# burakcuhadar/Photometric-Bundle-Adjustment

Hardware: AMD Instinct MI355X
Metric: photometric residual+jacobian blocks/sec (higher is better)
Workload: dtype f32; 1 GPU; C4: one synthetic problem of 1000 host keyframes x 100000 points x 8-px patch x 4 targets = 400000 residual blocks, 752x480 u8 images, pinhole; one step = full r + tangent-J evaluation (Ceres-mode records) at a new HBM-resident state; keyframes=1000, points=100000, patch=8, targets_per_point=4, blocks_total=400000, blocks_rank0=400000, parallelism=host-keyframe shards x1 (evaluation: no data-path collective; GN: one GPU)

## Files before the change

photometric-bundle-adjustment_amd/csrc/pba_engine.hip:

```cpp
#include <hip/hip_runtime.h>

#include <algorithm>
#include <chrono>
#include <cmath>
#include <cstdio>
#include <cstring>
#include <string>
#include <vector>

#include "pba_internal.h"
#include "pba_record.h"

using namespace pba;
using namespace pba::detail;

namespace pba {
namespace detail {
thread_local std::string g_last_error;
}
}

namespace {

__device__ __forceinline__ void make_pair(const double* __restrict__ poses, const int* __restrict__ pair_host,
// ... 530 lines not shown
  PBA_HIP(hipMemcpyAsync(e->block_point.p, block_point, n_blocks * sizeof(int), hipMemcpyHostToDevice, e->stream));
  PBA_HIP(hipMemcpyAsync(e->block_pair.p, pair_of.data(), n_blocks * sizeof(int), hipMemcpyHostToDevice, e->stream));
  std::vector<int2> pp(n_blocks);
  for (int b = 0; b < n_blocks; ++b) pp[b] = make_int2(block_point[b], pair_of[b]);
  PBA_HIP(e->block_pp.upload(pp, e->stream));
  PBA_HIP(hipMemcpyAsync(e->pair_host.p, ph.data(), np * sizeof(int), hipMemcpyHostToDevice, e->stream));
  PBA_HIP(hipMemcpyAsync(e->pair_target.p, pt.data(), np * sizeof(int), hipMemcpyHostToDevice, e->stream));
  if (geometric) {
    PBA_HIP(e->u_obs.resize(n_blocks));
    PBA_HIP(hipMemcpyAsync(e->u_obs.p, u_obs, n_blocks * sizeof(double2), hipMemcpyHostToDevice, e->stream));
  }
  PBA_HIP(e->out.resize((size_t)n_blocks * rec));
  PBA_HIP(e->cost.resize(n_blocks));
  PBA_HIP(e->valid.resize(n_blocks));
  PBA_HIP(hipStreamSynchronize(e->stream));
  e->n_blocks = n_blocks;
  e->n_pairs = np;
  e->evaluated = false;
  e->res_fresh = false;
  e->chunk_blocks = 0;
  e->n_chunks_async = 0;
  e->chunks_arrived.store(0);
  e->pairs_fresh = false;
  e->block_point_h.assign(block_point, block_point + n_blocks);
  e->block_target_h.assign(block_target, block_target + n_blocks);
  e->pair_of_h = std::move(pair_of);
  e->pair_host_h = std::move(ph);
  e->pair_target_h = std::move(pt);
  e->gn.prepared = false;
  e->aff.planned = false;
  e->aff.linearized = e->aff.have_step = false;
  e->joint.planned = e->joint.linearized = false;
  return upload_block_records(e);
}

int pba_set_state(pba_engine* e, const double* poses, const double* inv_dist) {
  if (!e || !poses || !inv_dist) return fail(PBA_ERR_INVALID_ARGUMENT, "null state");
  if (e->n_points <= 0 || e->n_frames <= 0) return fail(PBA_ERR_NOT_READY, "problem not set");
  if (int rc = check_device(e)) return rc;
  PBA_HIP(e->poses.resize(7 * (size_t)e->n_frames));
  PBA_HIP(hipMemcpyAsync(e->poses.p, poses, 7 * (size_t)e->n_frames * sizeof(double), hipMemcpyHostToDevice, e->stream));
  PBA_HIP(hipMemcpyAsync(e->rho.p, inv_dist, (size_t)e->n_points * sizeof(double), hipMemcpyHostToDevice, e->stream));
  e->state_set = true;
  e->pairs_fresh = false;
  e->joint.linearized = false;
  return PBA_OK;
}

int pba_set_state_device(pba_engine* e, const double* d_poses, const double* d_inv_dist) {
  if (!e || !d_poses || !d_inv_dist) return fail(PBA_ERR_INVALID_ARGUMENT, "null state");
  if (e->n_points <= 0 || e->n_frames <= 0) return fail(PBA_ERR_NOT_READY, "problem not set");
  if (int rc = check_device(e)) return rc;
  PBA_HIP(e->poses.resize(7 * (size_t)e->n_frames));
  const int n_pose_d = 7 * e->n_frames;
  const bool table = e->n_blocks > 0 && e->opt.residual_kind == PBA_RESIDUAL_GEOMETRIC;
  const int pair_wgs = table ? (e->n_pairs + 255) / 256 : 0;
  const int copy_wgs = std::min(1024, (std::max(n_pose_d, e->n_points) + 255) / 256);
  state_kernel<<<pair_wgs + copy_wgs, 256, 0, e->stream>>>(d_poses, d_inv_dist, e->poses.p, e->rho.p, n_pose_d,
                                                           e->n_points, e->pair_host.p, e->pair_target.p,
                                                           e->frame_cam.p, e->intr_d.p, e->pairs.p, e->n_pairs,
                                                           pair_wgs);
  PBA_HIP(hipGetLastError());
  e->state_set = true;
  e->pairs_fresh = table;
  e->joint.linearized = false;
  return PBA_OK;
}

namespace {

int evaluate_at(pba_engine* e, const double* poses, const double* rho, bool adopt, bool jac) {
  const bool photometric = e->opt.residual_kind == PBA_RESIDUAL_PHOTOMETRIC;
  if (photometric && (!e->have_images || e->P <= 0)) return fail(PBA_ERR_NOT_READY, "images/pattern missing");
  if (int rc = check_device(e)) return rc;
  KernelArgs ka;
  if (photometric) {
    const long long lanes = (long long)e->n_blocks * 8;
    if (adopt && lanes < std::max<long long>(7LL * e->n_frames, e->n_points)) {
      if (int rc = pba_set_state_device(e, poses, rho)) return rc;
      poses = e->poses.p;
      rho = e->rho.p;
      adopt = false;
    }
    ka = make_kernel_args(e, nullptr, rho);
    ka.poses = poses;
    if (adopt) {
      PBA_HIP(e->poses.resize(7 * (size_t)e->n_frames));
      ka.adopt_poses = e->poses.p;
      ka.adopt_rho = e->rho.p;
      e->state_set = true;
      e->pairs_fresh = false;
    }
  } else {
    if (adopt) {
      if (int rc = pba_set_state_device(e, poses, rho)) return rc;
    } else if (!e->pairs_fresh) {
      launch_pairs(e, e->poses.p, e->pairs.p);
    }
    e->pairs_fresh = true;
    ka = make_kernel_args(e, e->pairs.p, e->rho.p);
  }
  hipEvent_t ev_stop = nullptr;
  if (e->timing) {
    while (e->ev_pool.size() < e->ev_used + 2) {
      hipEvent_t ev;
      PBA_HIP(hipEventCreateWithFlags(&ev, hipEventDisableSystemFence));
      e->ev_pool.push_back(ev);
    }
    PBA_HIP(hipEventRecord(e->ev_pool[e->ev_used], e->stream));
    ev_stop = e->ev_pool[e->ev_used + 1];
    e->ev_used += 2;
  }
  if (!jac) {
    PBA_HIP(e->res.resize((size_t)e->n_blocks * e->R()));
    ka.res_out = e->res.p;
  }
  launch_mode(e, ka, jac ? 1 : 0);
  PBA_HIP(hipGetLastError());
  if (ev_stop) PBA_HIP(hipEventRecord(ev_stop, e->stream));
  e->evaluated = true;
  e->res_fresh = !jac;
  e->chunk_blocks = 0;
  e->n_chunks_async = 0;
  e->chunks_arrived.store(0);
  return PBA_OK;
}

}

int pba_evaluate(pba_engine* e, int32_t want_jacobians) {
  if (!e) return fail(PBA_ERR_INVALID_ARGUMENT, "null engine");
  if (e->n_blocks <= 0) return fail(PBA_ERR_NOT_READY, "pba_set_blocks first");
  if (!e->state_set) return fail(PBA_ERR_NOT_READY, "pba_set_state first");
  return evaluate_at(e, e->poses.p, e->rho.p, false, want_jacobians != 0);
}

int pba_evaluate_state_device(pba_engine* e, const double* d_poses, const double* d_inv_dist, int32_t want_jacobians) {
  if (!e || !d_poses || !d_inv_dist) return fail(PBA_ERR_INVALID_ARGUMENT, "null state");
  if (e->n_blocks <= 0) return fail(PBA_ERR_NOT_READY, "pba_set_blocks first");
  return evaluate_at(e, d_poses, d_inv_dist, true, want_jacobians != 0);
}

int pba_evaluate_states_device(pba_engine* e, int32_t n, const double* const* d_poses, const double* const* d_inv_dist,
                               int32_t want_jacobians) {
  if (!e || n < 0 || (n > 0 && (!d_poses || !d_inv_dist))) return fail(PBA_ERR_INVALID_ARGUMENT, "null states");
  if (e->n_blocks <= 0) return fail(PBA_ERR_NOT_READY, "pba_set_blocks first");
  for (int i = 0; i < n; ++i) {
    if (!d_poses[i] || !d_inv_dist[i]) return fail(PBA_ERR_INVALID_ARGUMENT, "null state");
    if (int rc = evaluate_at(e, d_poses[i], d_inv_dist[i], true, want_jacobians != 0)) return rc;
  }
  return PBA_OK;
}

int pba_enable_kernel_timing(pba_engine* e, int32_t enable) {
  if (!e) return fail(PBA_ERR_INVALID_ARGUMENT, "null engine");
  e->timing = enable != 0;
  return PBA_OK;
}

int pba_get_kernel_timing(pba_engine* e, double* total_ms, int32_t* launches) {
  if (!e || !total_ms) return fail(PBA_ERR_INVALID_ARGUMENT, "null argument");
  if (int rc = check_device(e)) return rc;
  PBA_HIP(hipStreamSynchronize(e->stream));
  double tot = 0;
  for (size_t i = 0; i + 1 < e->ev_used; i += 2) {
    float ms = 0;
    PBA_HIP(hipEventElapsedTime(&ms, e->ev_pool[i], e->ev_pool[i + 1]));
    tot += ms;
// ... 246 lines not shown
```

photometric-bundle-adjustment_amd/csrc/pba_evaluate.hip:

```cpp
#include <hip/hip_runtime.h>

#include <cmath>
#include <type_traits>

#include "pba_internal.h"
#include "pba_record.h"

using namespace pba;
using namespace pba::detail;

namespace {

template <int PM, int LPB, int MODE, class T>
__global__ __launch_bounds__(kBlockThreads) void photometric_block_kernel(const KernelArgs a) {
  constexpr int BPW = kBlockThreads / LPB;
  constexpr bool JAC = MODE == 1;
  using S = typename RecFormat<T>::S;
  constexpr int kCols = RecFormat<T>::kCols;
  constexpr int kStageBytes = JAC ? BPW * kCols * LPB * (int)sizeof(S) : 0;
  constexpr int kTileBytes = BPW * (int)sizeof(TileBlock);
  __shared__ __attribute__((aligned(16))) unsigned char lds[kStageBytes > kTileBytes ? kStageBytes : kTileBytes];
  TileBlock* s_tb = reinterpret_cast<TileBlock*>(lds);
  const int P = a.P;
  const int rec_f = kCols * P;
  const int blk0 = logical_tile() * BPW;
  const int lb = threadIdx.x / LPB;
  const int k = threadIdx.x % LPB;
  const int blk = blk0 + lb;
  const bool live = blk < a.n_blocks;
  const bool act = live && k < P;
  S* out = reinterpret_cast<S*>(a.out);

  const float2 off = pattern_at<LPB>(a, k);
  adopt_state(a);
  int pt;
  if (LPB == 8 && a.poses) {
    static_assert(kBlockThreads == 256, "stage_tile_wg: 4 waves, 32 blocks");
    pt = a.block_rec[live ? blk : a.n_blocks - 1].x;
    stage_tile_wg(a, s_tb, blk0);
  } else {
    pt = stage_tile<LPB>(a, s_tb, lb, k, blk, live);
  }
  const float Ih = act ? a.host_int[(long long)pt * P + k] : 0.0f;
  constexpr bool AFF = RecFormat<T>::kAffine;
  Affine af = {1.0f, 0.0f, 0.0f};
  if constexpr (AFF) af = block_affine(a, live ? blk : a.n_blocks - 1);
  __syncthreads();
  constexpr bool INTR = JAC && RecFormat<T>::kIntr;
  constexpr bool PFIN = RecFormat<T>::kIntr && AFF;
  float ji[8];
  const Row row = photometric_row<PM, JAC, TileBlock, false, INTR, AFF, PFIN>(a, s_tb[lb], off, Ih, nullptr, ji, &af);
  const int ok = group_all<LPB>(act ? row.ok : 1);
  const float s = group_sum<LPB>(act ? row.r * row.r : 0.0f);
  const float bc = ok ? huber_cost(s, a.huber) : 0.0f;
  if (live && k == 0) {
    a.valid[blk] = (uint8_t)ok;
    a.cost[blk] = bc;
  }
  if (MODE == 2) {
    if (a.wg_red) {
      const bool one = live && k == 0;
      wg_reduce2(one ? (double)bc : 0.0, one && ok ? 1.0 : 0.0, a.wg_red + 2 * logical_tile());
    }
    return;
  }
  if (!JAC) {
    if (act) {
      out[(long long)blk * rec_f + k] = rec_val<S>(ok ? row.r : 0.0f);
      if (a.res_out) a.res_out[(long long)blk * P + k] = ok ? row.r : 0.0f;
    }
    return;
  }
  __syncthreads();
  S* s_rec = reinterpret_cast<S*>(lds) + lb * rec_f;
  if constexpr (RecFormat<T>::kScaled) {
    stage_row_scaled(s_rec, lb, P, k, row, act && ok);
    if (act && !ok) {
      s_rec[k] = s_rec[col_jrho(P) + k] = s_rec[col_tail(P) + k] = (S)0.0f;
      for (int j = 0; j < 6; ++j) s_rec[col_jhost(P) + 6 * k + j] = s_rec[col_jtarget(P) + 6 * k + j] = (S)0.0f;
    }
  } else if (act) {
    if (ok) {
      stage_row_each<S>(s_rec, P, k, row);
    } else {
      S* h = s_rec + col_jhost(P) + 6 * k;
      S* t = s_rec + col_jtarget(P) + 6 * k;
      s_rec[k] = (S)0.0f;
      for (int j = 0; j < 6; ++j) h[j] = t[j] = (S)0.0f;
      s_rec[col_jrho(P) + k] = (S)0.0f;
    }
    if constexpr (INTR) {
      if (!ok) {
#pragma unroll
        for (int j = 0; j < 8; ++j) ji[j] = 0.0f;
      }
      stage_intr(s_rec, P, k, ji);
    }
    if constexpr (AFF) stage_affine<RecFormat<T>::kIntr>(s_rec, P, k, af.E * (Ih - af.bh), af.E, ok != 0);
  }
  __syncthreads();
  const int nblk = min(BPW, a.n_blocks - blk0);
  if (nblk <= 0) return;
  store_slab<S>(lds, reinterpret_cast<unsigned char*>(out + (long long)blk0 * rec_f), nblk * rec_f * (int)sizeof(S),
                a.slab_wt);
}

__host__ __device__ constexpr int multi_stage_bytes(int bpw, int P, int tsize, int cols = 14) {
  return (bpw * cols * P * tsize + 15) & ~15;
}

template <int PPL, class T>
constexpr int kMultiThreads = 32 * RecFormat<T>::kCols * 8 * PPL * (int)sizeof(typename RecFormat<T>::S) +
                                          32 * (int)sizeof(TileBlock) > 60 * 1024 ? 128 : 256;

template <int PPL, class T>
constexpr int kMultiWaves =
    RecFormat<T>::kIntr || RecFormat<T>::kAffine ? 3 : (RecFormat<T>::kScaled && PPL != 3 ? 5 : 6);
template <int PM, int PPL, class T>
constexpr int kMultiWavesPM = RecFormat<T>::kAffine && cam_of(PM) == CAM_KB4 ? 2 : kMultiWaves<PPL, T>;

template <int PM, int MODE, class T, int PPL, bool CT = false, bool C1 = false>
__global__ __launch_bounds__((kMultiThreads<PPL, T>))
__attribute__((amdgpu_waves_per_eu(CT ? (kMultiWavesPM<PM, PPL, T>) : 1, 8)))
void photometric_block_kernel_multi(const KernelArgs a) {
  constexpr int LPB = 8, NTH = kMultiThreads<PPL, T>, BPW = NTH / LPB;
  constexpr bool JAC = MODE == 1;
  static_assert(!CT || NTH == 256, "camera table: the workgroup-cooperative prologue");
  using TB = typename std::conditional<CT, TileBlockC, TileBlock>::type;
  extern __shared__ __attribute__((aligned(16))) unsigned char lds[];
  __shared__ float2 s_pat[LPB * PPL];
  __shared__ CamRec s_cam[CT ? kCamTab : 1];
  using S = typename RecFormat<T>::S;
  constexpr int kCols = RecFormat<T>::kCols;
  const int P = a.P;
  S* stage = reinterpret_cast<S*>(lds);
  TB* s_tb = reinterpret_cast<TB*>(lds + (JAC ? multi_stage_bytes(BPW, P, (int)sizeof(S), kCols) : 0));
  const int rec_f = kCols * P;
  const int blk0 = logical_tile() * BPW;
  const int lb = threadIdx.x / LPB;
  const int k = threadIdx.x % LPB;
  const int blk = blk0 + lb;
  const bool live = blk < a.n_blocks;
  S* out = reinterpret_cast<S*>(a.out);

  if ((int)threadIdx.x < LPB * PPL) s_pat[threadIdx.x] = pattern_at<LPB * PPL>(a, threadIdx.x);
  adopt_state(a);
  int pt;
  if constexpr (CT) {
    pt = a.block_rec[live ? blk : a.n_blocks - 1].x;
    stage_tile_wg_ct(a, s_tb, s_cam, a.n_cams, blk0);
  } else if (NTH == 256 && a.poses) {
    pt = a.block_rec[live ? blk : a.n_blocks - 1].x;
    stage_tile_wg(a, s_tb, blk0);
  } else {
    pt = stage_tile<LPB>(a, s_tb, lb, k, blk, live);
  }
  float Ih[PPL];
#pragma unroll
  for (int j = 0; j < PPL; ++j) {
    const int px = k + LPB * j;
    Ih[j] = live && px < P ? a.host_int[(long long)pt * P + px] : 0.0f;
  }
  constexpr bool AFF = RecFormat<T>::kAffine;
  Affine af = {1.0f, 0.0f, 0.0f};
  if constexpr (AFF) af = block_affine(a, live ? blk : a.n_blocks - 1);
  __syncthreads();
  S* s_rec = stage + lb * rec_f;
  int okl = 1;
  float s = 0.0f, rr[PPL];
  auto pixel = [&](int j, float ih) {
    const int px = k + LPB * j;
    const bool act = live && px < P;
    constexpr bool INTR = JAC && RecFormat<T>::kIntr;
    constexpr bool PFIN = RecFormat<T>::kIntr && AFF;
    float ji[8];
    const Row row =
        photometric_row<PM, JAC, TB, C1, INTR, AFF, PFIN>(a, s_tb[lb], s_pat[px < P ? px : 0], ih, s_cam, ji, &af);
    okl &= act ? row.ok : 1;
    s += act ? row.r * row.r : 0.0f;
    if constexpr (JAC && RecFormat<T>::kScaled) stage_row_scaled(s_rec, lb, P, px, row, act);
    else if constexpr (JAC) stage_row<S>(s_rec, P, px, row, act);
    if constexpr (INTR) {
      if (act) stage_intr(s_rec, P, px, ji);
    }
    if constexpr (JAC && AFF) {
      if (act) stage_affine<RecFormat<T>::kIntr>(s_rec, P, px, af.E * (ih - af.bh), af.E, true);
    }
// ... 168 lines not shown
  if ((reinterpret_cast<uintptr_t>(dst) & 15) == 0) {
    f32x4* d4 = reinterpret_cast<f32x4*>(dst);
    for (int i = threadIdx.x; i < (n_out >> 2); i += kBlockThreads)
      __builtin_nontemporal_store(f32x4{value(4 * i), value(4 * i + 1), value(4 * i + 2), value(4 * i + 3)}, d4 + i);
    for (int i = (n_out & ~3) + threadIdx.x; i < n_out; i += kBlockThreads) dst[i] = value(i);
  } else {
    for (int i = threadIdx.x; i < n_out; i += kBlockThreads) dst[i] = value(i);
  }
}

template <int MODEL>
void launch_geometric(pba_engine* e, const KernelArgs& ka, int mode) {
  const int grid = (e->n_blocks + kBlockThreads - 1) / kBlockThreads;
  e->last_grid = grid;
  if (mode == 1 && e->opt_intr) geometric_block_kernel<MODEL, true, true><<<grid, kBlockThreads, 0, e->stream>>>(ka);
  else if (mode == 1) geometric_block_kernel<MODEL, true, false><<<grid, kBlockThreads, 0, e->stream>>>(ka);
  else if (e->opt_intr) geometric_block_kernel<MODEL, false, true><<<grid, kBlockThreads, 0, e->stream>>>(ka);
  else geometric_block_kernel<MODEL, false, false><<<grid, kBlockThreads, 0, e->stream>>>(ka);
}

template <class T>
struct Tag { using type = T; };
template <int M>
using Mode = std::integral_constant<int, M>;

template <class F>
void dispatch_format(const pba_engine* e, int mode, F&& fn) {
  auto modes = [&](auto tag) {
    if (mode == 1) fn(tag, Mode<1>{});
    else if (mode == 0) fn(tag, Mode<0>{});
    else if constexpr (RecFormat<typename decltype(tag)::type>::kAffine) fn(Tag<AffineF32>{}, Mode<2>{});
    else fn(Tag<float>{}, Mode<2>{});
  };
  if (e->affine && e->opt_intr) modes(Tag<IntrAffineF32>{});
  else if (e->affine) modes(Tag<AffineF32>{});
  else if (e->opt_intr) modes(Tag<IntrF32>{});
  else if (e->record_format == PBA_RECORD_F16_SCALED) modes(Tag<ScaledF16>{});
  else if (e->record_format == PBA_RECORD_F16) modes(Tag<_Float16>{});
  else modes(Tag<float>{});
}

template <int PM, int M, class T>
void launch_block(pba_engine* e, KernelArgs ka) {
  const int grid = (int)(((long long)e->n_blocks * 8 + kBlockThreads - 1) / kBlockThreads);
  e->last_grid = grid;
  ka.slab_wt = grid <= kSlabWtGrid;
  photometric_block_kernel<PM, 8, M, T><<<grid, kBlockThreads, 0, e->stream>>>(ka);
}

template <int PM, int PPL, int M, class T>
void launch_multi(pba_engine* e, const KernelArgs& ka) {
  constexpr int nth = kMultiThreads<PPL, T>;
  const int grid = (int)(((long long)e->n_blocks * 8 + nth - 1) / nth);
  e->last_grid = grid;
  const size_t stage =
      M == 1 ? multi_stage_bytes(nth / 8, e->P, (int)sizeof(typename RecFormat<T>::S), RecFormat<T>::kCols) : 0;
  if constexpr (M == 1 && nth == 256) {
    if (ka.poses != nullptr && ka.n_cams <= kCamTab) {
      const size_t lds = stage + (size_t)(nth / 8) * sizeof(TileBlockC);
      if (ka.n_cams == 1) photometric_block_kernel_multi<PM, M, T, PPL, true, true><<<grid, nth, lds, e->stream>>>(ka);
      else photometric_block_kernel_multi<PM, M, T, PPL, true><<<grid, nth, lds, e->stream>>>(ka);
      return;
    }
  }
  photometric_block_kernel_multi<PM, M, T, PPL>
      <<<grid, nth, stage + (size_t)(nth / 8) * sizeof(TileBlock), e->stream>>>(ka);
}

template <int PM>
void launch_photometric(pba_engine* e, const KernelArgs& ka, int mode) {
  const int ppl = (e->P + 7) / 8;
  dispatch_format(e, mode, [&](auto tag, auto m) {
    using T = typename decltype(tag)::type;
    constexpr int M = decltype(m)::value;
    if (ppl <= 1) launch_block<PM, M, T>(e, ka);
    else if (ppl == 2) launch_multi<PM, 2, M, T>(e, ka);
    else if (ppl == 3) launch_multi<PM, 3, M, T>(e, ka);
    else launch_multi<PM, 4, M, T>(e, ka);
  });
}

}

namespace pba {
namespace detail {

void launch_mode(pba_engine* e, const KernelArgs& ka, int mode) {
  if (e->opt.residual_kind == PBA_RESIDUAL_GEOMETRIC) {
    switch (e->opt.camera_model) {
      case PBA_CAMERA_PINHOLE: launch_geometric<CAM_PINHOLE>(e, ka, mode); break;
      case PBA_CAMERA_DOUBLE_SPHERE: launch_geometric<CAM_DS>(e, ka, mode); break;
      case PBA_CAMERA_EUCM: launch_geometric<CAM_EUCM>(e, ka, mode); break;
      default: launch_geometric<CAM_KB4>(e, ka, mode); break;
    }
    return;
  }
  dispatch_pm(e, [&](auto pm) { launch_photometric<decltype(pm)::value>(e, ka, mode); });
}

KernelArgs make_kernel_args(pba_engine* e, const PairRec* pairs, const double* rho) {
  KernelArgs ka{};
  ka.images = e->images.p;
  ka.width = e->width;
  ka.height = e->height;
  ka.tiles_x = tiles_x_of(e->width);
  ka.frame_stride = tiled_frame_bytes(e->width, e->height);
  ka.umax = e->width + 1.0;
  ka.vmax = e->height + 1.0;
  ka.intr = e->intr.p;
  ka.intr_d = e->intr_d.p;
  ka.intr_t = e->opt_intr ? e->intr_state.p : e->intr.p;
  ka.intr_t_d = e->opt_intr ? e->intr_state_d.p : e->intr_d.p;
  ka.intr_scale = std::ldexp(1.0f, -e->level);
  ka.block_point = e->block_point.p;
  ka.block_pair = e->block_pair.p;
  ka.block_pp = e->block_pp.p;
  ka.pairs = pairs;
  ka.block_rec = e->block_rec.p;
  ka.n_pose_d = 7 * e->n_frames;
  ka.n_points = e->n_points;
  ka.u_ref = e->u_ref.p;
  ka.host_int = e->host_int.p;
  ka.rho = rho;
  ka.u_obs = e->u_obs.p;
  if (e->affine) ka.affine = e->affine_state.p;
  ka.out = e->out.p;
  ka.cost = e->cost.p;
  ka.valid = e->valid.p;
  ka.n_blocks = e->n_blocks;
  ka.n_cams = e->n_cams;
  ka.P = e->opt.residual_kind == PBA_RESIDUAL_PHOTOMETRIC ? e->P : 2;
  ka.huber = e->opt.huber_width;
  for (size_t i = 0; i < e->pattern_h.size() && i < 2 * PBA_MAX_PATTERN; ++i) ka.pattern[i] = e->pattern_h[i];
  return ka;
}

int launch_cost_only(pba_engine* e, const PairRec* pairs, const double* rho, double* wg_red, int* n_slots,
                     const double* poses, const float* intr_t, const double* intr_t_d, const double* affine) {
  KernelArgs ka = make_kernel_args(e, pairs, rho);
  ka.poses = poses;
  if (affine && e->affine) ka.affine = affine;
  if (intr_t) ka.intr_t = intr_t;
  if (intr_t_d) ka.intr_t_d = intr_t_d;
  ka.wg_red = wg_red;
  launch_mode(e, ka, 2);
  if (n_slots) *n_slots = e->last_grid;
  PBA_HIP(hipGetLastError());
  return PBA_OK;
}

int launch_decode_records(pba_engine* e, float* d_out) {
  if (e->record_format == PBA_RECORD_F32) {
    PBA_HIP(hipMemcpyAsync(d_out, e->out.p, (size_t)e->n_blocks * e->rec_floats() * sizeof(float),
                           hipMemcpyDeviceToDevice, e->stream));
    return PBA_OK;
  }
  const int grid = (e->n_blocks + kDecodeBlocks - 1) / kDecodeBlocks;
  const bool scaled = e->record_format == PBA_RECORD_F16_SCALED;
  decode_records_kernel<<<grid, kBlockThreads, 0, e->stream>>>(
      reinterpret_cast<const _Float16*>(e->out.p), d_out, e->n_blocks, e->P,
      scaled ? (int)RecFormat<ScaledF16>::kCols : (int)RecFormat<_Float16>::kCols);
  PBA_HIP(hipGetLastError());
  return PBA_OK;
}

}
// ... 2 lines not shown
```

photometric-bundle-adjustment_amd/csrc/pba_internal.h:

```cpp
#pragma once

#include <hip/hip_runtime.h>

#include <algorithm>
#include <cstdint>
#include <cstdlib>
#include <type_traits>
#include <string>
#include <vector>

#include "pba.h"
#include "pba_device.h"
#include "pba_host.h"

namespace pba {
namespace detail {

inline const char* test_hook(const char* name) {
#ifdef PBA_TEST_HOOKS
  return std::getenv(name);
#else
  (void)name;
  return nullptr;
#endif
// ... 307 lines not shown
  return ((m >> sh) & grp) == grp;
}

struct Row {
  float r = 0.0f, jr = 0.0f;
  Vec3 hv = {0, 0, 0}, hw = {0, 0, 0}, tv = {0, 0, 0}, tw = {0, 0, 0};
  int ok = 1;
};

template <int LPB>
__device__ __forceinline__ int stage_tile_pp(const KernelArgs& a, TileBlock* s_tb, int lb, int k, int2 pp);
template <int LPB>
__device__ __forceinline__ int stage_tile(const KernelArgs& a, TileBlock* s_tb, int lb, int k, int blk, bool live) {
  uint4* dst = reinterpret_cast<uint4*>(s_tb + lb);
  if (LPB >= 8 && a.poses) {
    static_assert(kCamK == 8, "fused prologue: 8 camera parts");
    const int4 br = a.block_rec[live ? blk : a.n_blocks - 1];
    const double* H = a.poses + 7 * br.y;
    const double* T = a.poses + 7 * br.z;
    double h[7], t[7];
#pragma unroll
    for (int j = 0; j < 7; ++j) {
      h[j] = H[j];
      t[j] = T[j];
    }
    const int hc = br.w >> 16, tc = br.w & 0xffff, kc = k & 7;
    const uint4 cam = reinterpret_cast<const uint4*>(kc < 4 ? a.intr_d + kCamD * hc + kCamHk : a.intr_t_d + kCamD * tc)[kc & 3];
    const uint4 ur = reinterpret_cast<const uint4*>(a.u_ref)[br.x];
    const double rho = a.rho[br.x];
    asm volatile("" ::"v"(cam.x), "v"(cam.y), "v"(cam.z), "v"(cam.w), "v"(ur.x), "v"(ur.y), "v"(ur.z), "v"(ur.w),
                 "v"(rho));
#pragma unroll
    for (int j = 0; j < 7; ++j) asm volatile("" ::"v"(h[j]), "v"(t[j]));
    PairRec& pr = s_tb[lb].pr;
    if (k < 8) dst[(int)(offsetof(PairRec, hk) / 16) + k] = cam;
    if (k >= 4 && k < 8) camera_kf_part(cam, k - 4, pr.kf);
    if (k == 0) {
      pair_rotation(h, t, pr);
    } else if (k == 1) {
      pair_translation(h, t, pr);
      pr.host_cam = hc;
      pr.target_cam = tc;
      pr.target = br.z;
      pr.host = br.y;
    } else if (k == 2) {
      dst[kPairParts] = ur;
    } else if (k == 3) {
      const long long img = (long long)br.z * a.frame_stride;
      dst[kPairParts + 1] = make_uint4(__double2loint(rho), __double2hiint(rho), (unsigned)img, (unsigned)(img >> 32));
    }
    return br.x;
  }
  return stage_tile_pp<LPB>(a, s_tb, lb, k, a.block_pp[live ? blk : a.n_blocks - 1]);
}

template <int LPB>
__device__ __forceinline__ int stage_tile_pp(const KernelArgs& a, TileBlock* s_tb, int lb, int k, int2 pp) {
  constexpr int NP = (kTileParts + LPB - 1) / LPB;
  uint4* dst = reinterpret_cast<uint4*>(s_tb + lb);
  const uint4* src = reinterpret_cast<const uint4*>(a.pairs + pp.y);
  uint4 v[NP];
#pragma unroll
  for (int i = 0; i < NP; ++i) {
    const int part = k + LPB * i;
    v[i] = part == kPairParts ? reinterpret_cast<const uint4*>(a.u_ref)[pp.x] : src[part < kPairParts ? part : 0];
  }
  const double r = a.rho[pp.x];
  const int tgt = a.pairs[pp.y].target;
  asm volatile("" ::"v"(r), "v"(tgt));
#pragma unroll
  for (int i = 0; i < NP; ++i) asm volatile("" ::"v"(v[i].x), "v"(v[i].y), "v"(v[i].z), "v"(v[i].w));
#pragma unroll
  for (int i = 0; i < NP; ++i) {
    const int part = k + LPB * i;
    if (part == kPairParts + 1) {
      const long long img = (long long)tgt * a.frame_stride;
      v[i] = make_uint4(__double2loint(r), __double2hiint(r), (unsigned)img, (unsigned)(img >> 32));
    }
    if (part < kTileParts) dst[part] = v[i];
  }
  return pp.x;
}

__device__ __forceinline__ void stage_tile_wg(const KernelArgs& a, TileBlock* s_tb, int blk0) {
  const int w = threadIdx.x >> 6, lane = threadIdx.x & 63, b = lane & 31;
  const int4 br = a.block_rec[min(blk0 + b, a.n_blocks - 1)];
  PairRec& pr = s_tb[b].pr;
  uint4* dst = reinterpret_cast<uint4*>(s_tb + b);
  if (w == 0) {
    if (lane < 32) {
      const double* H = a.poses + 7 * br.y;
      const double* T = a.poses + 7 * br.z;
      double h[4], t[4];
#pragma unroll
      for (int j = 0; j < 4; ++j) {
        h[j] = H[j];
        t[j] = T[j];
      }
      pair_rotation(h, t, pr);
    }
  } else if (w == 1) {
    if (lane < 32) {
      const double* H = a.poses + 7 * br.y;
      const double* T = a.poses + 7 * br.z;
      double h[7], t[7];
#pragma unroll
      for (int j = 0; j < 7; ++j) {
        h[j] = H[j];
        t[j] = T[j];
      }
      pair_translation(h, t, pr);
      pr.host_cam = br.w >> 16;
      pr.target_cam = br.w & 0xffff;
      pr.target = br.z;
      pr.host = br.y;
    }
  } else if (w == 2) {
    const bool tgt = lane >= 32;
    const uint4* src = reinterpret_cast<const uint4*>(tgt ? a.intr_t_d + kCamD * (br.w & 0xffff) : a.intr_d + kCamD * (br.w >> 16) + kCamHk);
    uint4 c[4];
#pragma unroll
    for (int q = 0; q < 4; ++q) c[q] = src[q];
    uint4* d = dst + (int)(offsetof(PairRec, hk) / 16) + (tgt ? 4 : 0);
#pragma unroll
    for (int q = 0; q < 4; ++q) d[q] = c[q];
    if (tgt) {
#pragma unroll
      for (int q = 0; q < 4; ++q) camera_kf_part(c[q], q, pr.kf);
    }
  } else {
    if (lane < 32) {
      dst[kPairParts] = reinterpret_cast<const uint4*>(a.u_ref)[br.x];
    } else {
      const double rho = a.rho[br.x];
      const long long img = (long long)br.z * a.frame_stride;
      dst[kPairParts + 1] = make_uint4(__double2loint(rho), __double2hiint(rho), (unsigned)img, (unsigned)(img >> 32));
    }
  }
}

__device__ __forceinline__ void stage_tile_wg_ct(const KernelArgs& a, TileBlockC* s_tb, CamRec* s_cam, int n_cams,
                                                 int blk0) {
  const int w = threadIdx.x >> 6, lane = threadIdx.x & 63, b = lane & 31;
  const int4 br = a.block_rec[min(blk0 + b, a.n_blocks - 1)];
  TileBlockC& tb = s_tb[b];
  if (w == 0) {
    if (lane < 32) {
      const double* H = a.poses + 7 * br.y;
      const double* T = a.poses + 7 * br.z;
      double h[4], t[4];
#pragma unroll
      for (int j = 0; j < 4; ++j) {
        h[j] = H[j];
        t[j] = T[j];
      }
      pair_rotation(h, t, tb);
    }
  } else if (w == 1) {
    if (lane < 32) {
      const double* H = a.poses + 7 * br.y;
      const double* T = a.poses + 7 * br.z;
      double h[7], t[7];
#pragma unroll
      for (int j = 0; j < 7; ++j) {
        h[j] = H[j];
        t[j] = T[j];
      }
      pair_translation(h, t, tb);
      tb.host_cam = br.w >> 16;
      tb.target_cam = br.w & 0xffff;
      tb.target = br.z;
      tb.host = br.y;
    }
  } else if (w == 2) {
    const int c = lane >> 3, q = lane & 7;
    if (c < n_cams) {
      const uint4 v = reinterpret_cast<const uint4*>(q < 4 ? a.intr_d + kCamD * c + kCamHk : a.intr_t_d + kCamD * c)[q & 3];
      uint4* d = reinterpret_cast<uint4*>(s_cam + c);
      d[q] = v;
      if (q >= 4) camera_kf_part(v, q - 4, s_cam[c].kf);
    }
  } else {
    if (lane < 32) {
      tb.ur = a.u_ref[br.x];
    } else {
      tb.rho = a.rho[br.x];
      tb.img = (long long)br.z * a.frame_stride;
    }
  }
}

template <int N>
__device__ __forceinline__ float2 pattern_at(const KernelArgs& a, int k) {
  float2 o = make_float2(a.pattern[0], a.pattern[1]);
#pragma unroll
  for (int j = 1; j < N; ++j)
    if (k == j) o = make_float2(a.pattern[2 * j], a.pattern[2 * j + 1]);
  return o;
}

__device__ __forceinline__ void adopt_state(const KernelArgs& a) {
  if (!a.adopt_rho) return;
  const long long g = (long long)blockIdx.x * blockDim.x + threadIdx.x;
  if (g >= a.n_points && g >= a.n_pose_d) return;
  const double r = a.rho[g < a.n_points ? g : 0], p = a.poses[g < a.n_pose_d ? g : 0];
  asm volatile("" ::"v"(r), "v"(p));
  if (g < a.n_points) a.adopt_rho[g] = r;
  if (g < a.n_pose_d) a.adopt_poses[g] = p;
}

struct Affine {
  float E, bh, bt;
};
__device__ __forceinline__ Affine block_affine(const KernelArgs& a, int blk, int pair = -1) {
  int h, t;
  if (pair < 0 && a.poses) {
    const int4 br = a.block_rec[blk];
    h = br.y;
    t = br.z;
  } else {
    const PairRec& pr = a.pairs[pair >= 0 ? pair : a.block_pp[blk].y];
    h = pr.host;
    t = pr.target;
  }
  const double2 ah = reinterpret_cast<const double2*>(a.affine)[h];
  const double2 at = reinterpret_cast<const double2*>(a.affine)[t];
  const double d = at.x - ah.x;
  const double E = isfinite(ah.x) && isfinite(at.x) ? exp(d) : __builtin_nan("");
  return {(float)E, (float)ah.y, (float)at.y};
}

template <int PM, bool JAC, class TB = TileBlock, bool C1 = false, bool INTR = false, bool AFF = false,
          bool PFIN = false>
__device__ __forceinline__ Row photometric_row(const KernelArgs& a, const TB& tb, float2 off, float Ih,
                                               const CamRec* tab = nullptr, float* ji = nullptr,
                                               const Affine* af = nullptr) {
  constexpr int MODEL = cam_of(PM);
  Row o;
  const auto& pp = pose_of(tb);
  const CamView cv = C1 ? single_camera(a) : cams_of(tb, tab);
  const double rho = tb.rho;
  const Vec3d b = unproject<MODEL>(cv.hk, tb.ur.x + (double)off.x, tb.ur.y + (double)off.y);
  const Vec3d Rb = mat_mul(pp.R, b);
  const Vec3d p = {Rb.x + rho * pp.t[0], Rb.y + rho * pp.t[1], Rb.z + rho * pp.t[2]};
  const bool dom = in_domain<MODEL>(cv.tk, p);
  float I, gx, gy;
  double u, v;
  const double iden = project<MODEL>(cv.tk, p, u, v);
  interpolate<interp_of(PM)>(a.images + tb.img, a.umax, a.vmax, a.tiles_x, u, v, I, gx, gy);
  if (AFF) o.r = (I - af->bt) - af->E * (Ih - af->bh);
  else o.r = I - Ih;
  o.ok = dom && isfinite(o.r);
  if constexpr (PFIN) o.ok = o.ok && isfinite(u) && isfinite(v);
  if (JAC) {
    const Vec3 pf = to_f(p), bf = to_f(b);
    Vec3 du, dv;
    project_jac<MODEL>(cv.kf, pf, (float)iden, du, dv);
    const Vec3 q = {gx * du.x + gy * dv.x, gx * du.y + gy * dv.y, gx * du.z + gy * dv.z};
    const Vec3 qR = row_mul(q, pp.Rf);
    const float rf = (float)rho;
    o.hv = {rf * qR.x, rf * qR.y, rf * qR.z};
    o.hw = cross(bf, qR);
    o.tv = {-rf * q.x, -rf * q.y, -rf * q.z};
    o.tw = cross(q, pf);
    if (MODEL == CAM_PINHOLE) {
      const double ex = fma(-(p.x * iden), pp.t[2], pp.t[0]), ey = fma(-(p.y * iden), pp.t[2], pp.t[1]);
      o.jr = (float)(iden * fma((double)gx * cv.tk[0], ex, (double)gy * cv.tk[1] * ey));
    } else {
      Vec3d dud, dvd;
      project_jac<MODEL>(cv.tk, p, iden, dud, dvd);
      const Vec3d td = {pp.t[0], pp.t[1], pp.t[2]};
      o.jr = (float)((double)gx * dot(dud, td) + (double)gy * dot(dvd, td));
    }
    if (INTR) {
      float ku[8], kv[8];
      if (MODEL == CAM_KB4)
        project_intr_jac_kb4(cv.kf, pf, (float)iden, (float)atan2(sqrt(p.x * p.x + p.y * p.y), p.z), ku, kv);
      else
        project_intr_jac<MODEL>(cv.kf, pf, (float)iden, ku, kv);
#pragma unroll
      for (int j = 0; j < 8; ++j) ji[j] = (gx * ku[j] + gy * kv[j]) * (j < 4 ? a.intr_scale : 1.0f);
// ... 418 lines not shown
```

photometric-bundle-adjustment_amd/csrc/pba_record.h:

```cpp
#pragma once

#include <type_traits>

#include "pba_internal.h"

namespace {

struct ScaledF16 {};
struct IntrF32 {};
struct AffineF32 {};
struct IntrAffineF32 {};
template <class Stored, int Cols, bool Scaled = false, bool Intr = false, bool Affine = false>
struct RecLayout {
  using S = Stored;
  static constexpr int kCols = Cols;
  static constexpr bool kScaled = Scaled, kIntr = Intr, kAffine = Affine;
};
template <class T>
struct RecFormat : RecLayout<T, 14> {};
template <>
struct RecFormat<ScaledF16> : RecLayout<_Float16, 15, true> {};
template <>
struct RecFormat<IntrF32> : RecLayout<float, 22, false, true> {};
template <>
struct RecFormat<AffineF32> : RecLayout<float, 18, false, false, true> {};
template <>
struct RecFormat<IntrAffineF32> : RecLayout<float, 26, false, true, true> {};

}

namespace pba {
namespace detail {

__host__ __device__ __forceinline__ constexpr int col_r(int) { return 0; }
__host__ __device__ __forceinline__ constexpr int col_jhost(int P) { return P; }
__host__ __device__ __forceinline__ constexpr int col_jtarget(int P) { return 7 * P; }
__host__ __device__ __forceinline__ constexpr int col_jrho(int P) { return 13 * P; }
__host__ __device__ __forceinline__ constexpr int col_tail(int P) { return 14 * P; }
template <bool INTR = false>
__host__ __device__ __forceinline__ constexpr int col_jab_host(int P) {
  if constexpr (INTR) return col_tail(P) + 8 * P;
  else return col_tail(P);
}
template <bool INTR = false>
__host__ __device__ __forceinline__ constexpr int col_jab_target(int P) {
  if constexpr (INTR) return col_tail(P) + 10 * P;
  else return col_tail(P) + 2 * P;
}

__host__ __device__ __forceinline__ constexpr int scale_row_of(int c, int P) {
  return c < col_jhost(P) ? -1 : c < col_jrho(P) ? ((c - col_jhost(P)) % (6 * P)) / 6 : c - col_jrho(P);
}

template <class T>
__device__ __forceinline__ T rec_val(float v) { return (T)v; }
template <>
__device__ __forceinline__ _Float16 rec_val<_Float16>(float v) {
  return (_Float16)(isnan(v) ? v : __builtin_amdgcn_fmed3f(v, -65504.0f, 65504.0f));
}

template <bool INTR = false>
__device__ __forceinline__ void stage_affine(float* s_rec, int P, int px, float g, float E, bool ok) {
  reinterpret_cast<float2*>(s_rec + col_jab_host<INTR>(P))[px] = ok ? make_float2(g, E) : make_float2(0.0f, 0.0f);
  reinterpret_cast<float2*>(s_rec + col_jab_target<INTR>(P))[px] = ok ? make_float2(-g, -1.0f) : make_float2(0.0f, 0.0f);
}

__device__ __forceinline__ void stage_intr(float* s_rec, int P, int px, const float (&ji)[8]) {
  float* d = s_rec + col_tail(P) + 8 * px;
  if ((P & 1) == 0) {
    reinterpret_cast<f32x4*>(d)[0] = f32x4{ji[0], ji[1], ji[2], ji[3]};
    reinterpret_cast<f32x4*>(d)[1] = f32x4{ji[4], ji[5], ji[6], ji[7]};
  } else {
#pragma unroll
    for (int q = 0; q < 4; ++q) reinterpret_cast<float2*>(d)[q] = make_float2(ji[2 * q], ji[2 * q + 1]);
  }
}

template <class T, int NTH = kBlockThreads>
__device__ __forceinline__ void store_slab(const unsigned char* src, unsigned char* dst, int bytes, int wt = 0) {
  constexpr int kBlockThreads = NTH;
  if ((((uintptr_t)dst | (unsigned)bytes) & 15) == 0) {
    const f32x4* s4 = reinterpret_cast<const f32x4*>(src);
    f32x4* d4 = reinterpret_cast<f32x4*>(dst);
    if (wt) {
      for (int i = threadIdx.x; i < (bytes >> 4); i += kBlockThreads)
        asm volatile("global_store_dwordx4 %0, %1, off nt sc1" ::"v"(d4 + i), "v"(s4[i]) : "memory");
    } else {
      for (int i = threadIdx.x; i < (bytes >> 4); i += kBlockThreads) __builtin_nontemporal_store(s4[i], d4 + i);
    }
  } else if (sizeof(T) == 4 || (((uintptr_t)dst | (unsigned)bytes) & 3) == 0) {
    const float* s1 = reinterpret_cast<const float*>(src);
    float* d1 = reinterpret_cast<float*>(dst);
#pragma unroll 1
    for (int i = threadIdx.x; i < (bytes >> 2); i += kBlockThreads) __builtin_nontemporal_store(s1[i], d1 + i);
  } else {
    const _Float16* s1 = reinterpret_cast<const _Float16*>(src);
    _Float16* d1 = reinterpret_cast<_Float16*>(dst);
#pragma unroll 1
    for (int i = threadIdx.x; i < (bytes >> 1); i += kBlockThreads) d1[i] = s1[i];
  }
}

typedef float rec_f2 __attribute__((ext_vector_type(2)));
typedef _Float16 rec_h2 __attribute__((ext_vector_type(2)));

__device__ __forceinline__ void stage_halves(_Float16* s_rec, int P, int px, const rec_h2 (&c)[7], bool even) {
  _Float16* h = s_rec + col_jhost(P) + 6 * px;
  _Float16* t = s_rec + col_jtarget(P) + 6 * px;
  s_rec[col_r(P) + px] = c[0].x;
  s_rec[col_jrho(P) + px] = c[0].y;
  if (even) {
    rec_h2* h4 = reinterpret_cast<rec_h2*>(h);
    rec_h2* t4 = reinterpret_cast<rec_h2*>(t);
    h4[0] = c[1]; h4[1] = c[2]; h4[2] = c[3];
    t4[0] = c[4]; t4[1] = c[5]; t4[2] = c[6];
  } else {
    rec_h2* h4 = reinterpret_cast<rec_h2*>(h + 1);
    rec_h2* t4 = reinterpret_cast<rec_h2*>(t + 1);
    h[0] = c[1].x; h4[0] = (rec_h2){c[1].y, c[2].x}; h4[1] = (rec_h2){c[2].y, c[3].x}; h[5] = c[3].y;
    t[0] = c[4].x; t4[0] = (rec_h2){c[4].y, c[5].x}; t4[1] = (rec_h2){c[5].y, c[6].x}; t[5] = c[6].y;
  }
}

__device__ __forceinline__ void stage_row_scaled(_Float16* s_rec, int lb, int P, int px, const Row& row, bool act) {
  const float j[13] = {row.jr, row.hv.x, row.hv.y, row.hv.z, row.hw.x, row.hw.y, row.hw.z,
                       row.tv.x, row.tv.y, row.tv.z, row.tw.x, row.tw.y, row.tw.z};
  float m = 0.0f;
#pragma unroll
  for (int q = 0; q < 13; ++q) m = fmaxf(m, fabsf(j[q]));
  int ex = 0;
  if (m >= 65520.0f) ex = min((int)((__float_as_uint(m) >> 23) & 0xffu) - (127 + 14), 15);
  const float inv = __uint_as_float((unsigned)(127 - ex) << 23);
  const float r = isnan(row.r) ? row.r : __builtin_amdgcn_fmed3f(row.r, -65504.0f, 65504.0f);
  rec_h2 c[7];
  c[0] = __builtin_convertvector((rec_f2){r, j[0] * inv}, rec_h2);
#pragma unroll
  for (int q = 1; q < 7; ++q) c[q] = __builtin_convertvector((rec_f2){j[2 * q - 1] * inv, j[2 * q] * inv}, rec_h2);
  if (ex == 15) {
    auto sat = [](_Float16 h) -> _Float16 {
      return __builtin_isinf(h) ? (h > (_Float16)0 ? (_Float16)65504.0f : (_Float16)-65504.0f) : h;
    };
    c[0].y = sat(c[0].y);
#pragma unroll
    for (int q = 1; q < 7; ++q) c[q] = (rec_h2){sat(c[q].x), sat(c[q].y)};
  }
  if (act) {
    stage_halves(s_rec, P, px, c, ((lb + 1) & P & 1) == 0);
    reinterpret_cast<unsigned short*>(s_rec)[col_tail(P) + px] = (unsigned short)((15 + ex) << 10);
  }
}

template <class T>
__device__ __forceinline__ void stage_row_each(T* s_rec, int P, int px, const Row& row) {
  T* h = s_rec + col_jhost(P) + 6 * px;
  T* t = s_rec + col_jtarget(P) + 6 * px;
  s_rec[col_r(P) + px] = rec_val<T>(row.r);
  h[0] = rec_val<T>(row.hv.x); h[1] = rec_val<T>(row.hv.y); h[2] = rec_val<T>(row.hv.z);
  h[3] = rec_val<T>(row.hw.x); h[4] = rec_val<T>(row.hw.y); h[5] = rec_val<T>(row.hw.z);
  t[0] = rec_val<T>(row.tv.x); t[1] = rec_val<T>(row.tv.y); t[2] = rec_val<T>(row.tv.z);
  t[3] = rec_val<T>(row.tw.x); t[4] = rec_val<T>(row.tw.y); t[5] = rec_val<T>(row.tw.z);
  s_rec[col_jrho(P) + px] = rec_val<T>(row.jr);
}

template <class T>
__device__ __forceinline__ void stage_row(T* s_rec, int P, int px, const Row& row, bool act) {
  if constexpr (std::is_same<T, _Float16>::value) {
    typedef rec_f2 f2;
    typedef rec_h2 h2;
    const float v[14] = {row.r, row.jr, row.hv.x, row.hv.y, row.hv.z, row.hw.x, row.hw.y, row.hw.z,
                         row.tv.x, row.tv.y, row.tv.z, row.tw.x, row.tw.y, row.tw.z};
    h2 c[7];
    float m = 0.0f;
#pragma unroll
    for (int q = 0; q < 7; ++q) {
      c[q] = __builtin_convertvector((f2){v[2 * q], v[2 * q + 1]}, h2);
      m = fmaxf(m, fmaxf(fabsf(v[2 * q]), fabsf(v[2 * q + 1])));
    }
    const bool big = m >= 65520.0f;
    if (__ballot(act && big) != 0) {
      auto sat = [](_Float16 h) -> _Float16 {
        return __builtin_isinf(h) ? (h > (_Float16)0 ? (_Float16)65504.0f : (_Float16)-65504.0f) : h;
      };
// ... 12 lines not shown
```

Before: 8.720 billion blocks/s.

## Give each wave a private LDS region to drop workgroup barriers in record staging

Reorganizes the per-block photometric kernel's LDS into per-wave regions, each holding that wave's 8 tile blocks and staged records. Each wave then stores its own slab slice, so the two __syncthreads around record staging become compiler barriers only. The block record load is hoisted and shared via shuffle, and pattern offsets are pinned to scalar registers. It also adds optional timestamp instrumentation and a test-only pair-table path. The risk is that wave-local stores are narrower (64 threads), and correctness depends on no cross-wave LDS sharing after the tile stage.

```diff
diff --git a/photometric-bundle-adjustment_amd/csrc/pba_engine.hip b/photometric-bundle-adjustment_amd/csrc/pba_engine.hip
--- a/photometric-bundle-adjustment_amd/csrc/pba_engine.hip
+++ b/photometric-bundle-adjustment_amd/csrc/pba_engine.hip
@@ -636,8 +636,20 @@
       rho = e->rho.p;
       adopt = false;
     }
-    ka = make_kernel_args(e, nullptr, rho);
-    ka.poses = poses;
+    if (test_hook("PBA_TEST_PAIR_TABLE")) {
+      if (adopt) {
+        if (int rc = pba_set_state_device(e, poses, rho)) return rc;
+        poses = e->poses.p;
+        rho = e->rho.p;
+        adopt = false;
+      }
+      launch_pairs(e, poses, e->pairs.p);
+      e->pairs_fresh = false;
+      ka = make_kernel_args(e, e->pairs.p, rho);
+    } else {
+      ka = make_kernel_args(e, nullptr, rho);
+      ka.poses = poses;
+    }
     if (adopt) {
       PBA_HIP(e->poses.resize(7 * (size_t)e->n_frames));
       ka.adopt_poses = e->poses.p;
diff --git a/photometric-bundle-adjustment_amd/csrc/pba_evaluate.hip b/photometric-bundle-adjustment_amd/csrc/pba_evaluate.hip
--- a/photometric-bundle-adjustment_amd/csrc/pba_evaluate.hip
+++ b/photometric-bundle-adjustment_amd/csrc/pba_evaluate.hip
@@ -10,6 +10,22 @@
 using namespace pba::detail;
 
 namespace {
+
+#ifdef PBA_EVAL_STAMPS
+constexpr int kEvalStamps = 9;
+__device__ long long* g_eval_stamps = nullptr;
+#define PBA_STAMP(i, wait_loads)                                        \
+  do {                                                                  \
+    if (wait_loads) asm volatile("s_waitcnt vmcnt(0)" ::: "memory");    \
+    __builtin_amdgcn_sched_barrier(0);                                  \
+    stamps[i] = wall_clock64();                                         \
+    __builtin_amdgcn_sched_barrier(0);                                  \
+  } while (0)
+#else
+#define PBA_STAMP(i, wait_loads) \
+  do {                           \
+  } while (0)
+#endif
 
 template <int PM, int LPB, int MODE, class T>
 __global__ __launch_bounds__(kBlockThreads) void photometric_block_kernel(const KernelArgs a) {
@@ -17,42 +33,71 @@
   constexpr bool JAC = MODE == 1;
   using S = typename RecFormat<T>::S;
   constexpr int kCols = RecFormat<T>::kCols;
-  constexpr int kStageBytes = JAC ? BPW * kCols * LPB * (int)sizeof(S) : 0;
-  constexpr int kTileBytes = BPW * (int)sizeof(TileBlock);
-  __shared__ __attribute__((aligned(16))) unsigned char lds[kStageBytes > kTileBytes ? kStageBytes : kTileBytes];
-  TileBlock* s_tb = reinterpret_cast<TileBlock*>(lds);
+  static_assert(LPB == kSlabMaxPattern && BPW == kSlabWaves * kSlabWaveBlocks && sizeof(TileBlock) == kSlabTileBytes,
+                "pba_wave_slab.h: 4 waves of 8 blocks, 8 lanes each");
+  static_assert(slab_format_known(kCols, (int)sizeof(S)), "pba_wave_slab.h: kSlabFormats has no entry for this format");
+  constexpr int kRegion = wave_region_bytes(kCols, (int)sizeof(S), JAC);
+  __shared__ __attribute__((aligned(16))) unsigned char lds[wg_lds_bytes(kCols, (int)sizeof(S), JAC)];
+  auto tile_at = [&](int b) { return reinterpret_cast<TileBlock*>(lds + tile_block_offset(b, kRegion)); };
+  const int w = __builtin_amdgcn_readfirstlane(threadIdx.x / 64);
+  unsigned char* const region = lds + wave_region_offset(w, kRegion);
   const int P = a.P;
   const int rec_f = kCols * P;
   const int blk0 = logical_tile() * BPW;
-  const int lb = threadIdx.x / LPB;
+  const int wb = (threadIdx.x / LPB) % kSlabWaveBlocks;
+  const int lb = w * kSlabWaveBlocks + wb;
   const int k = threadIdx.x % LPB;
   const int blk = blk0 + lb;
   const bool live = blk < a.n_blocks;
   const bool act = live && k < P;
+  TileBlock* const own_tile = reinterpret_cast<TileBlock*>(region + wb * kSlabTileBytes);
   S* out = reinterpret_cast<S*>(a.out);
 
+#ifdef PBA_EVAL_STAMPS
+  long long stamps[kEvalStamps] = {};
+#endif
+  PBA_STAMP(0, false);
   const float2 off = pattern_at<LPB>(a, k);
   adopt_state(a);
   int pt;
+  float Ih;
+  auto host_intensity = [&]() { return act ? a.host_int[(long long)pt * P + k] : 0.0f; };
   if (LPB == 8 && a.poses) {
     static_assert(kBlockThreads == 256, "stage_tile_wg: 4 waves, 32 blocks");
-    pt = a.block_rec[live ? blk : a.n_blocks - 1].x;
-    stage_tile_wg(a, s_tb, blk0);
+    const int4 br = tile_block_rec(a, blk0);
+#ifdef PBA_EVAL_STAMPS
+    asm volatile("" ::"v"(br.x));
+    PBA_STAMP(1, true);
+#endif
+    pt = __shfl(br.x, lb, 64);
+    Ih = host_intensity();
+    stage_tile_wg(a, tile_at, br);
   } else {
-    pt = stage_tile<LPB>(a, s_tb, lb, k, blk, live);
-  }
-  const float Ih = act ? a.host_int[(long long)pt * P + k] : 0.0f;
+    pt = stage_tile<LPB>(a, own_tile, 0, k, blk, live);
+    Ih = host_intensity();
+  }
   constexpr bool AFF = RecFormat<T>::kAffine;
   Affine af = {1.0f, 0.0f, 0.0f};
   if constexpr (AFF) af = block_affine(a, live ? blk : a.n_blocks - 1);
+  PBA_STAMP(2, true);
   __syncthreads();
+  PBA_STAMP(3, false);
+#ifdef PBA_EVAL_STAMPS
+  asm volatile("" ::"v"(Ih));
+  PBA_STAMP(4, true);
+#endif
   constexpr bool INTR = JAC && RecFormat<T>::kIntr;
   constexpr bool PFIN = RecFormat<T>::kIntr && AFF;
   float ji[8];
-  const Row row = photometric_row<PM, JAC, TileBlock, false, INTR, AFF, PFIN>(a, s_tb[lb], off, Ih, nullptr, ji, &af);
+  const Row row =
+      photometric_row<PM, JAC, TileBlock, false, INTR, AFF, PFIN>(a, *own_tile, off, Ih, nullptr, ji, &af);
   const int ok = group_all<LPB>(act ? row.ok : 1);
   const float s = group_sum<LPB>(act ? row.r * row.r : 0.0f);
   const float bc = ok ? huber_cost(s, a.huber) : 0.0f;
+#ifdef PBA_EVAL_STAMPS
+  asm volatile("" ::"v"(bc));
+  PBA_STAMP(5, false);
+#endif
   if (live && k == 0) {
     a.valid[blk] = (uint8_t)ok;
     a.cost[blk] = bc;
@@ -71,8 +116,9 @@
     }
     return;
   }
-  __syncthreads();
-  S* s_rec = reinterpret_cast<S*>(lds) + lb * rec_f;
+  asm volatile("" ::: "memory");
+  PBA_STAMP(6, false);
+  S* s_rec = reinterpret_cast<S*>(region + wb * rec_f * (int)sizeof(S));
   if constexpr (RecFormat<T>::kScaled) {
     stage_row_scaled(s_rec, lb, P, k, row, act && ok);
     if (act && !ok) {
@@ -98,11 +144,18 @@
     }
     if constexpr (AFF) stage_affine<RecFormat<T>::kIntr>(s_rec, P, k, af.E * (Ih - af.bh), af.E, ok != 0);
   }
-  __syncthreads();
+  asm volatile("" ::: "memory");
+  PBA_STAMP(7, false);
   const int nblk = min(BPW, a.n_blocks - blk0);
   if (nblk <= 0) return;
-  store_slab<S>(lds, reinterpret_cast<unsigned char*>(out + (long long)blk0 * rec_f), nblk * rec_f * (int)sizeof(S),
-                a.slab_wt);
+  const WaveStore ws = wave_store_range(w, nblk, rec_f * (int)sizeof(S));
+  store_slab<S, 64>(region, reinterpret_cast<unsigned char*>(out + (long long)blk0 * rec_f) + ws.begin,
+                    ws.bytes, a.slab_wt, threadIdx.x % 64);
+#ifdef PBA_EVAL_STAMPS
+  PBA_STAMP(8, true);
+  if (threadIdx.x == 0 && g_eval_stamps)
+    for (int i = 0; i < kEvalStamps; ++i) g_eval_stamps[16LL * blockIdx.x + i] = stamps[i];
+#endif
 }
 
 __host__ __device__ constexpr int multi_stage_bytes(int bpw, int P, int tsize, int cols = 14) {
@@ -437,6 +490,12 @@
 
 }
 
+#ifdef PBA_EVAL_STAMPS
+extern "C" int pba_test_set_eval_stamps(long long* d_stamps) {
+  return hipMemcpyToSymbol(HIP_SYMBOL(g_eval_stamps), &d_stamps, sizeof(d_stamps)) == hipSuccess ? 0 : -1;
+}
+#endif
+
 namespace pba {
 namespace detail {
 
diff --git a/photometric-bundle-adjustment_amd/csrc/pba_internal.h b/photometric-bundle-adjustment_amd/csrc/pba_internal.h
--- a/photometric-bundle-adjustment_amd/csrc/pba_internal.h
+++ b/photometric-bundle-adjustment_amd/csrc/pba_internal.h
@@ -413,11 +413,16 @@
   return pp.x;
 }
 
-__device__ __forceinline__ void stage_tile_wg(const KernelArgs& a, TileBlock* s_tb, int blk0) {
+__device__ __forceinline__ int4 tile_block_rec(const KernelArgs& a, int blk0) {
+  const int b = threadIdx.x & 31;
+  return a.block_rec[min(blk0 + b, a.n_blocks - 1)];
+}
+template <class Place>
+__device__ __forceinline__ void stage_tile_wg(const KernelArgs& a, Place tile_at, const int4 br) {
   const int w = threadIdx.x >> 6, lane = threadIdx.x & 63, b = lane & 31;
-  const int4 br = a.block_rec[min(blk0 + b, a.n_blocks - 1)];
-  PairRec& pr = s_tb[b].pr;
-  uint4* dst = reinterpret_cast<uint4*>(s_tb + b);
+  TileBlock* const tb = tile_at(b);
+  PairRec& pr = tb->pr;
+  uint4* dst = reinterpret_cast<uint4*>(tb);
   if (w == 0) {
     if (lane < 32) {
       const double* H = a.poses + 7 * br.y;
@@ -468,6 +473,10 @@
       dst[kPairParts + 1] = make_uint4(__double2loint(rho), __double2hiint(rho), (unsigned)img, (unsigned)(img >> 32));
     }
   }
+}
+
+__device__ __forceinline__ void stage_tile_wg(const KernelArgs& a, TileBlock* s_tb, int blk0) {
+  stage_tile_wg(a, [=](int b) { return s_tb + b; }, tile_block_rec(a, blk0));
 }
 
 __device__ __forceinline__ void stage_tile_wg_ct(const KernelArgs& a, TileBlockC* s_tb, CamRec* s_cam, int n_cams,
@@ -523,11 +532,19 @@
 
 template <int N>
 __device__ __forceinline__ float2 pattern_at(const KernelArgs& a, int k) {
-  float2 o = make_float2(a.pattern[0], a.pattern[1]);
-#pragma unroll
-  for (int j = 1; j < N; ++j)
-    if (k == j) o = make_float2(a.pattern[2 * j], a.pattern[2 * j + 1]);
-  return o;
+  typedef float pat2 __attribute__((ext_vector_type(2)));
+  auto pinned = [&](int j) {
+    pat2 v = {a.pattern[2 * j], a.pattern[2 * j + 1]};
+    asm("" : "+s"(v));
+    return v;
+  };
+  pat2 o = pinned(0);
+#pragma unroll
+  for (int j = 1; j < N; ++j) {
+    const pat2 p = pinned(j);
+    o = k == j ? p : o;
+  }
+  return make_float2(o.x, o.y);
 }
 
 __device__ __forceinline__ void adopt_state(const KernelArgs& a) {
diff --git a/photometric-bundle-adjustment_amd/csrc/pba_record.h b/photometric-bundle-adjustment_amd/csrc/pba_record.h
--- a/photometric-bundle-adjustment_amd/csrc/pba_record.h
+++ b/photometric-bundle-adjustment_amd/csrc/pba_record.h
@@ -3,6 +3,7 @@
 #include <type_traits>
 
 #include "pba_internal.h"
+#include "pba_wave_slab.h"
 
 namespace {
 
@@ -27,6 +28,15 @@
 template <>
 struct RecFormat<IntrAffineF32> : RecLayout<float, 26, false, true, true> {};
 
+template <class T>
+constexpr bool slab_entry_is(int i) {
+  return pba::detail::kSlabFormats[i].cols == RecFormat<T>::kCols &&
+         pba::detail::kSlabFormats[i].ssize == (int)sizeof(typename RecFormat<T>::S);
+}
+static_assert(slab_entry_is<float>(0) && slab_entry_is<_Float16>(1) && slab_entry_is<ScaledF16>(2) &&
+                  slab_entry_is<IntrF32>(3) && slab_entry_is<AffineF32>(4) && slab_entry_is<IntrAffineF32>(5),
+              "pba_wave_slab.h: kSlabFormats");
+
 }
 
 namespace pba {
@@ -77,27 +87,28 @@
 }
 
 template <class T, int NTH = kBlockThreads>
-__device__ __forceinline__ void store_slab(const unsigned char* src, unsigned char* dst, int bytes, int wt = 0) {
+__device__ __forceinline__ void store_slab(const unsigned char* src, unsigned char* dst, int bytes, int wt = 0,
+                                           int tid = threadIdx.x) {
   constexpr int kBlockThreads = NTH;
   if ((((uintptr_t)dst | (unsigned)bytes) & 15) == 0) {
     const f32x4* s4 = reinterpret_cast<const f32x4*>(src);
     f32x4* d4 = reinterpret_cast<f32x4*>(dst);
     if (wt) {
-      for (int i = threadIdx.x; i < (bytes >> 4); i += kBlockThreads)
+      for (int i = tid; i < (bytes >> 4); i += kBlockThreads)
         asm volatile("global_store_dwordx4 %0, %1, off nt sc1" ::"v"(d4 + i), "v"(s4[i]) : "memory");
     } else {
-      for (int i = threadIdx.x; i < (bytes >> 4); i += kBlockThreads) __builtin_nontemporal_store(s4[i], d4 + i);
+      for (int i = tid; i < (bytes >> 4); i += kBlockThreads) __builtin_nontemporal_store(s4[i], d4 + i);
     }
   } else if (sizeof(T) == 4 || (((uintptr_t)dst | (unsigned)bytes) & 3) == 0) {
     const float* s1 = reinterpret_cast<const float*>(src);
     float* d1 = reinterpret_cast<float*>(dst);
 #pragma unroll 1
-    for (int i = threadIdx.x; i < (bytes >> 2); i += kBlockThreads) __builtin_nontemporal_store(s1[i], d1 + i);
+    for (int i = tid; i < (bytes >> 2); i += kBlockThreads) __builtin_nontemporal_store(s1[i], d1 + i);
   } else {
     const _Float16* s1 = reinterpret_cast<const _Float16*>(src);
     _Float16* d1 = reinterpret_cast<_Float16*>(dst);
 #pragma unroll 1
-    for (int i = threadIdx.x; i < (bytes >> 1); i += kBlockThreads) d1[i] = s1[i];
+    for (int i = tid; i < (bytes >> 1); i += kBlockThreads) d1[i] = s1[i];
   }
 }
 
diff --git a/photometric-bundle-adjustment_amd/csrc/pba_wave_slab.h b/photometric-bundle-adjustment_amd/csrc/pba_wave_slab.h
--- /dev/null
+++ b/photometric-bundle-adjustment_amd/csrc/pba_wave_slab.h
@@ -0,0 +1,56 @@
+#pragma once
+
+#if defined(__HIPCC__) || defined(__CUDACC__)
+#define PBA_HD __host__ __device__
+#else
+#define PBA_HD
+#endif
+
+namespace pba {
+namespace detail {
+
+constexpr int kSlabWaves = 4;
+constexpr int kSlabWaveBlocks = 8;
+constexpr int kSlabMaxPattern = 8;
+constexpr int kSlabTileBytes = 352;
+
+struct SlabFormat {
+  const char* name;
+  int cols, ssize;
+};
+constexpr SlabFormat kSlabFormats[] = {{"f32", 14, 4},  {"f16", 14, 2},    {"scaled", 15, 2},
+                                       {"intr", 22, 4}, {"affine", 18, 4}, {"intr_affine", 26, 4}};
+constexpr int kSlabFormatCount = (int)(sizeof(kSlabFormats) / sizeof(kSlabFormats[0]));
+PBA_HD constexpr bool slab_format_known(int cols, int ssize) {
+  for (int i = 0; i < kSlabFormatCount; ++i)
+    if (kSlabFormats[i].cols == cols && kSlabFormats[i].ssize == ssize) return true;
+  return false;
+}
+
+PBA_HD constexpr int wave_region_bytes(int cols, int ssize, bool records = true) {
+  const int tile = kSlabWaveBlocks * kSlabTileBytes;
+  const int stage = records ? kSlabWaveBlocks * cols * kSlabMaxPattern * ssize : 0;
+  return stage > tile ? stage : tile;
+}
+PBA_HD constexpr int wg_lds_bytes(int cols, int ssize, bool records = true) {
+  return kSlabWaves * wave_region_bytes(cols, ssize, records);
+}
+PBA_HD constexpr int wave_region_offset(int w, int region) { return w * region; }
+PBA_HD constexpr int tile_block_offset(int lb, int region) {
+  return wave_region_offset(lb / kSlabWaveBlocks, region) + (lb % kSlabWaveBlocks) * kSlabTileBytes;
+}
+PBA_HD constexpr int staged_record_offset(int lb, int region, int rec_bytes) {
+  return wave_region_offset(lb / kSlabWaveBlocks, region) + (lb % kSlabWaveBlocks) * rec_bytes;
+}
+
+struct WaveStore {
+  int begin, bytes;
+};
+PBA_HD constexpr WaveStore wave_store_range(int w, int nblk, int rec_bytes) {
+  const int first = w * kSlabWaveBlocks;
+  const int n = nblk - first < 0 ? 0 : (nblk - first > kSlabWaveBlocks ? kSlabWaveBlocks : nblk - first);
+  return {first * rec_bytes, n * rec_bytes};
+}
+
+}
+}
```

New measurement: 8.843 billion blocks/s (median of 6 runs). +1.4%, better.
